# FarrOutLab/GWInferno

Hardware: AMD Instinct MI355X
Metric: log-likelihood evals/sec (value + gradient + diagnostic sites, host theta -> host results) (higher is better)
Workload: dtype f64; 1 GPU; C2: PL+Peak m1 x PL q x PL z, 69 ev x 5000 PE x 50k inj; n_events=69, n_pe=5000, n_inj=50000, n_theta=6, parallelism=single GPU

## Files before the change

### gwinferno_amd/csrc/gwi_device.h

```cpp
#pragma once
#ifndef __HIPCC_RTC__
#include <hip/hip_runtime.h>
#endif

#include "gwi_engine.h"

namespace gwi {

constexpr int kBlock = 256;
constexpr int kWaves = kBlock / 64;
constexpr int kMaxDerived = 7;
constexpr int kRecHeader = 3;

struct TermD {
  int kind, n_basis;
  int th0, th1, th2, th3;
  int flags, th4;
  double p0, p1, p2;
  double p3;
};
static_assert(sizeof(TermD) == 64, "twelve of these sit in the 4 KiB kernel-argument block");

struct NormD {
  int n_pts, expo_theta, n_basis, coef_off, flags, pad;
// ... 897 lines not shown
  }
  __device__ static void init(Acc& a) {
#pragma unroll
    for (int j = 0; j < 5; ++j) a.g[j] = 0;
  }
  __device__ static void rescale(Acc& a, double sc) {
#pragma unroll
    for (int j = 0; j < 5; ++j) a.g[j] *= sc;
  }
  static constexpr int kNumAcc = 5;
  __device__ static void collect(const TermD& t, const Acc& a, double* vals, int* th) {
#pragma unroll
    for (int j = 0; j < 5; ++j) vals[j] = a.g[j];
    th[0] = t.th0;
    th[1] = t.th1;
    th[2] = t.th2;
    th[3] = t.th3;
    th[4] = t.th4;
  }
};

template <>
struct Absorbs<GWI_TERM_PLPEAK> {
  static constexpr bool value = true;
};
template <>
struct Absorbs<GWI_TERM_PLPEAK_SMOOTH> {
  static constexpr bool value = true;
};

template <>
struct Term<GWI_TERM_POWERLAW_BOUNDS> {
  static constexpr bool kSpline = false;
  struct In {
    double x0, x1;
  };
  __device__ static void load(const double* const* tc, SIdx idx, In& in) {
    in.x0 = gload(tc[0], idx);
    in.x1 = gload(tc[1], idx);
  }
  struct State {
    double lx;
  };
  struct Acc {
    double g0;
  };
  __device__ static double eval(const TermD& t, const double*, const Ctx& c, const In& in, State& s, double& lin) {
    s.lx = in.x0;
    if ((in.x1 < c.theta[t.th1]) || (in.x1 > c.theta[t.th2])) {
      lin = 0.0;
      s.lx = 0.0;
    }
    return c.theta[t.th0] * s.lx;
  }
  __device__ static void accumulate(const TermD&, const Ctx&, double w, const State& s, Acc& a) { a.g0 += w * s.lx; }
  GWI_ACC1(g0)
  static constexpr int kNumAcc = 1;
  __device__ static void collect(const TermD& t, const Acc& a, double* vals, int* th) {
    vals[0] = a.g0;
    th[0] = t.th0;
  }
};

template <>
struct Term<GWI_TERM_EXP_SPLINE_LERP> {
  static constexpr bool kSpline = true;
  struct In {
    double x0;
  };
  __device__ static void load(const double* const* tc, SIdx idx, In& in) { in.x0 = gload(tc[0], idx); }
  struct State {
    double t0, t1, f;
    int k0, k1;
  };
  struct Acc {};
  __device__ static double node(const TermD& t, const Ctx& c, double sx, double wt, int& k, double& tt, double& lin) {
    spline_locate_x(sx, t, k, tt);
    double v = spline_value(c, t.th0 + k, tt);
    if (!((sx >= t.p0) && (sx <= t.p1))) {
      k = -1;
      v = 0.0;
      if (!(t.flags & GWI_SPLINE_OUTSIDE_ZERO_EXPONENT) && wt != 0.0) lin = 0.0;
    }
    if (wt == 0.0) k = -1;
    return v;
  }
  __device__ static double eval(const TermD& t, const double*, const Ctx& c, const In& in, State& s, double& lin) {
    const NormD& nd = c.a->norms[t.th1];
    const double u = in.x0;
    int j = (int)u;
    j = max(0, min(j, nd.n_pts - 2));
    const double f = u - (double)j;
    const double s0 = gload(nd.us, j), s1 = gload(nd.us, j + 1);
    const double l0 = node(t, c, s0, 1.0 - f, s.k0, s.t0, lin);
    const double l1 = node(t, c, s1, f, s.k1, s.t1, lin);
    s.f = f;
    return fma(f, l1 - l0, l0);
  }
  __device__ static void accumulate(const TermD& t, const Ctx& c, double w, const State& s, Acc&) {
    if (w != 0.0) {
      if (s.k0 >= 0) spline_scatter(c, t.th0 + s.k0, cubic_taps_weighted(s.t0, make_weight(w * (1.0 - s.f))));
      if (s.k1 >= 0) spline_scatter(c, t.th0 + s.k1, cubic_taps_weighted(s.t1, make_weight(w * s.f)));
    }
  }
  __device__ static void init(Acc&) {}
  __device__ static void rescale(Acc&, double) {}
  static constexpr int kNumAcc = 0;
  __device__ static void collect(const TermD&, const Acc&, double*, int*) {}
};

template <int U, bool TAKEN, int... Ks>
struct ChainImpl;
template <int U, bool TAKEN>
struct ChainImpl<U, TAKEN> {
  static constexpr bool kGeneric = false;
  static constexpr bool kSpline = false;
  static constexpr bool kAbsorb = false;
  static constexpr int kNumAcc = 0;
  __device__ void init() {}
  __device__ void load(int, int, int, const Ctx&, SIdx) {}
  __device__ void advance() {}
  __device__ double eval(int, int, const Ctx&, double&) { return 0.0; }
  __device__ double finish(int, int, const Ctx&, double, double, int) { return 0.0; }
  __device__ void accumulate(int, int, const Ctx&, double, double) {}
  __device__ void rescale(double) {}
  __device__ void collect(int, const Ctx&, double*, int*) {}
};
template <int U, bool TAKEN, int K, int... Rest>
struct ChainImpl<U, TAKEN, K, Rest...> {
  static constexpr bool kDefer = !TAKEN && Absorbs<K>::value;
  using RestT = ChainImpl<U, TAKEN || kDefer, Rest...>;
  static constexpr bool kGeneric = false;
  static constexpr bool kSpline = Term<K>::kSpline || RestT::kSpline;
  static constexpr bool kAbsorb = kDefer || RestT::kAbsorb;
  static constexpr int kNumAcc = Term<K>::kNumAcc + RestT::kNumAcc;
  typename Term<K>::In in[2][U];
  typename Term<K>::State st[U];
  typename Term<K>::Acc acc;
  RestT rest;
  __device__ void init() {
    Term<K>::init(acc);
    rest.init();
  }
  __device__ void load(int buf, int u, int ti, const Ctx& c, SIdx idx) {
    Term<K>::load(c.tcols[ti], idx, in[buf][u]);
    rest.load(buf, u, ti + 1, c, idx);
  }
  __device__ void advance() {
#pragma unroll
    for (int u = 0; u < U; ++u) in[0][u] = in[1][u];
    rest.advance();
  }
  __device__ double eval(int u, int ti, const Ctx& c, double& lin) {
    if constexpr (kDefer) {
      return rest.eval(u, ti + 1, c, lin);
    } else {
      const double l = Term<K>::eval(c.a->terms[ti], c.derived[ti], c, in[0][u], st[u], lin);
      return l + rest.eval(u, ti + 1, c, lin);
    }
  }
  __device__ double finish(int u, int ti, const Ctx& c, double L, double E, int nshift) {
    if constexpr (kDefer)
      return Term<K>::finish(c.a->terms[ti], c.derived[ti], c, in[0][u], st[u], L, E, nshift);
    else
      return rest.finish(u, ti + 1, c, L, E, nshift);
  }
  __device__ void accumulate(int u, int ti, const Ctx& c, double w, double wfac) {
    if constexpr (kDefer)
      Term<K>::accumulate_weighted(wfac, st[u], acc);
    else
      Term<K>::accumulate(c.a->terms[ti], c, w, st[u], acc);
    rest.accumulate(u, ti + 1, c, w, wfac);
  }
  __device__ void rescale(double sc) {
    Term<K>::rescale(acc, sc);
    rest.rescale(sc);
  }
  __device__ void collect(int ti, const Ctx& c, double* vals, int* th) {
    Term<K>::collect(c.a->terms[ti], acc, vals, th);
    rest.collect(ti + 1, c, vals + Term<K>::kNumAcc, th + Term<K>::kNumAcc);
  }
};

constexpr int kGenericChain = 0;
#define GWI_FOR_EACH_KIND(X)                                                                                             \
  X(GWI_TERM_POWERLAW) X(GWI_TERM_PLPEAK) X(GWI_TERM_POWERLAW_RATIO) X(GWI_TERM_BETA) X(GWI_TERM_TILT_MIXTURE)           \
  X(GWI_TERM_POWERLAW_REDSHIFT) X(GWI_TERM_EXP_SPLINE) X(GWI_TERM_TRUNCNORM) X(GWI_TERM_LINEAR_SPLINE) X(GWI_TERM_TILT_JOINT) \
  X(GWI_TERM_SMOOTH) X(GWI_TERM_PLPEAK_SMOOTH) X(GWI_TERM_POWERLAW_BOUNDS) X(GWI_TERM_EXP_SPLINE_LERP) X(GWI_TERM_EXP_SPLINE_F32)        \
  X(GWI_TERM_LINEAR_SPLINE_F32)
template <int K>
__device__ __forceinline__ double generic_value(const TermD& t, const double* d, const Ctx& c, const double* const* tc, SIdx idx, double& lin) {
  typename Term<K>::In in;
  typename Term<K>::State st;
  Term<K>::load(tc, idx, in);
  return Term<K>::eval(t, d, c, in, st, lin);
}
template <int K>
__device__ __forceinline__ void generic_gradient(const TermD& t, const double* d, const Ctx& c, const double* const* tc, SIdx idx, double w) {
  typename Term<K>::In in;
  typename Term<K>::State st;
  typename Term<K>::Acc acc;
  Term<K>::load(tc, idx, in);
  double lin = 1.0;
  Term<K>::eval(t, d, c, in, st, lin);
  Term<K>::init(acc);
  Term<K>::accumulate(t, c, w, st, acc);
  constexpr int kN = Term<K>::kNumAcc;
  if constexpr (kN > 0) {
    double vals[kN];
    int th[kN];
    Term<K>::collect(t, acc, vals, th);
#pragma unroll
    for (int j = 0; j < kN; ++j)
      if (vals[j] != 0.0) unsafeAtomicAdd(c.gacc + (th[j] << c.rep_shift), vals[j]);
  }
}
template <int U>
struct ChainImpl<U, false, kGenericChain> {
  static constexpr bool kGeneric = true;
  static constexpr bool kSpline = true;
  static constexpr bool kAbsorb = false;
  static constexpr int kNumAcc = 0;
  SIdx idx[2][U];
  __device__ void init() {}
  __device__ void load(int buf, int u, int, const Ctx&, SIdx i) { idx[buf][u] = i; }
  __device__ void advance() {
#pragma unroll
    for (int u = 0; u < U; ++u) idx[0][u] = idx[1][u];
  }
  __device__ double eval(int u, int, const Ctx& c, double& lin) {
    double l = 0.0;
    for (int t = 0; t < c.a->n_terms; ++t) {
      const TermD& td = c.a->terms[t];
      switch (td.kind) {
#define GWI_X(K) \
  case K: l += generic_value<K>(td, c.derived[t], c, c.tcols[t], idx[0][u], lin); break;
        GWI_FOR_EACH_KIND(GWI_X)
#undef GWI_X
        default: lin = 0.0;
      }
    }
    return l;
  }
  __device__ double finish(int, int, const Ctx&, double, double, int) { return 0.0; }
  __device__ void accumulate(int u, int, const Ctx& c, double w, double) {
    if (w == 0.0) return;
    c.wt = make_weight(w);
    for (int t = 0; t < c.a->n_terms; ++t) {
      const TermD& td = c.a->terms[t];
      switch (td.kind) {
#define GWI_X(K) \
  case K: generic_gradient<K>(td, c.derived[t], c, c.tcols[t], idx[0][u], w); break;
        GWI_FOR_EACH_KIND(GWI_X)
#undef GWI_X
        default: break;
      }
    }
  }
  __device__ void rescale(double) {}
  __device__ void collect(int, const Ctx&, double*, int*) {}
};

template <int U, int... Ks>
using Chain = ChainImpl<U, false, Ks...>;


__device__ __forceinline__ void store_sys(double* p, double v) { __hip_atomic_store(p, v, __ATOMIC_RELAXED, __HIP_MEMORY_SCOPE_SYSTEM); }
__device__ __forceinline__ void publish_stamp(double* slot, unsigned long long seq, int tid) {
  asm volatile("s_waitcnt vmcnt(0)" ::: "memory");
  __syncthreads();
  if (tid == 0) __hip_atomic_store(reinterpret_cast<unsigned long long*>(slot), seq, __ATOMIC_RELAXED, __HIP_MEMORY_SCOPE_SYSTEM);
}
__device__ __forceinline__ double lane_bcast(double v, int src) {
  const int lo = __builtin_amdgcn_readlane(__double2loint(v), src);
  const int hi = __builtin_amdgcn_readlane(__double2hiint(v), src);
  return __hiloint2double(hi, lo);
}

__device__ __forceinline__ double load_fresh(const double* p) { return __hip_atomic_load(p, __ATOMIC_RELAXED, __HIP_MEMORY_SCOPE_SYSTEM); }
__device__ __forceinline__ void combine_group(const TailArgs& a, const int e, const int kb, const int tid) {
  const int lane = tid & 63;
  const bool is_inj = e >= a.n_ev;
  int n_tiles;
  long long first;
  if (is_inj) {
    const int j = e - a.n_ev;
    const int t0 = j * a.tiles_per_inj_group;
    n_tiles = a.n_inj_tiles - t0 < a.tiles_per_inj_group ? a.n_inj_tiles - t0 : a.tiles_per_inj_group;
    first = (long long)a.n_ev * a.tiles_per_event + t0;
  } else {
    n_tiles = a.tiles_per_event;
    first = (long long)e * a.tiles_per_event;
  }
  const int n_groups = a.n_ev + a.n_inj_groups;
  const double* rec = a.partials + ((long long)kb * a.n_scan_blocks + first) * a.rec_stride;
  double* const ev_out = a.ev_out + (long long)kb * a.n_ev * 4;
  double* const ev_grad = a.ev_grad + (long long)kb * a.n_ev * a.n_theta;
  double* const inj_out = a.inj_out + (long long)kb * a.n_inj_groups * 4;
  double* const inj_grad = a.inj_grad + (long long)kb * a.n_inj_groups * a.n_theta;
  double* const ev_host = a.ev_host + (long long)kb * 3 * a.n_ev;
  const int row_doubles = 8 * a.row_lines;
  double* const host_rows = a.host_rows ? a.host_rows + (long long)kb * n_groups * row_doubles : nullptr;
  __shared__ double s_row[4 + GWI_MAX_THETA];

  const bool has = lane < n_tiles;
  const double* mine = rec + (long long)(has ? lane : 0) * a.rec_stride;
  const double m_t = has ? load_fresh(mine) : GWI_NEG_INF;
  const double r1 = has ? load_fresh(mine + 1) : 0.0, r2 = has ? load_fresh(mine + 2) : 0.0;
  constexpr int kEarly = 16;
  double early[kEarly];
  const bool early_on = tid < a.n_theta;
  {
    const double* col0 = rec + kRecHeader + (early_on ? tid : 0);
#pragma unroll
    for (int t = 0; t < kEarly; ++t) early[t] = (early_on && t < n_tiles) ? load_fresh(col0 + (long long)t * a.rec_stride) : 0.0;
  }
  const double M = wave_max(m_t);
  const double f = (m_t == GWI_NEG_INF) ? 0.0 : exp(m_t - M);
  const double S1 = wave_sum(f * r1);
  const double inv_s1 = S1 > 0.0 ? 1.0 / S1 : 0.0;
  for (int p = tid; p < a.n_theta; p += a.combine_threads) {
    double acc = 0.0;
    const double* col = rec + kRecHeader + p;
    int t = 0;
    if (p == tid) {
#pragma unroll
      for (; t < kEarly; ++t)
        if (t < n_tiles) acc += lane_bcast(f, t) * early[t];
      t = n_tiles < kEarly ? n_tiles : kEarly;
    }
#pragma unroll 4
    for (; t < n_tiles; ++t) acc += lane_bcast(f, t) * load_fresh(col + (long long)t * a.rec_stride);
    if (host_rows)
      s_row[3 + p] = is_inj ? acc : acc * inv_s1;
    else if (is_inj)
      inj_grad[(long long)(e - a.n_ev) * a.n_theta + p] = acc;
    else
      ev_grad[(long long)e * a.n_theta + p] = acc * inv_s1;
  }
  if (tid < 64) {
    const double S2 = wave_sum(f * f * r2);
    if (lane == 0 && host_rows) {
      if (is_inj) {
        s_row[0] = M;
        s_row[1] = S1;
        s_row[2] = S2;
      } else {
        const double log_s1 = log(S1);
        const double log_neff = 2.0 * log_s1 - log(S2);
        s_row[0] = log_s1 + M;
        s_row[1] = log_neff;
        s_row[2] = 1.0 / exp(log_neff) - 1.0 / a.n_pe;
      }
    } else if (lane == 0) {
      if (is_inj) {
        double* o = inj_out + (long long)(e - a.n_ev) * 4;
        o[0] = M;
        o[1] = S1;
        o[2] = S2;
      } else {
        const double log_s1 = log(S1);
        const double log_neff = 2.0 * log_s1 - log(S2);
        const double var = 1.0 / exp(log_neff) - 1.0 / a.n_pe;
        double* o = ev_out + (long long)e * 4;
        o[0] = log_s1 + M;
        o[1] = log_neff;
        o[2] = var;
        o[3] = S1;
        if (a.publish_events) {
          store_sys(ev_host + e, log_s1 + M);
          store_sys(ev_host + a.n_ev + e, log_neff);
          store_sys(ev_host + 2 * a.n_ev + e, var);
        }
      }
    }
  }
  if (host_rows) {
    __syncthreads();
    unsigned long long* o = reinterpret_cast<unsigned long long*>(host_rows + (long long)e * row_doubles);
    const unsigned long long seq = __hip_atomic_load(a.seq_ptr, __ATOMIC_RELAXED, __HIP_MEMORY_SCOPE_SYSTEM);
    const int n_vals = 3 + a.n_theta;
    for (int slot = tid; slot < row_doubles; slot += a.combine_threads) {
      const int line = slot >> 3, j = slot & 7, i = line * 7 + j;
      const unsigned long long bits = j == 7 ? seq : (i < n_vals ? (unsigned long long)__double_as_longlong(s_row[i]) : 0ull);
      __hip_atomic_store(o + slot, bits, __ATOMIC_RELAXED, __HIP_MEMORY_SCOPE_SYSTEM);
    }
  }
}

__device__ __forceinline__ int pow2_at_least(int v) {
  int p = 1;
  while (p < v) p <<= 1;
  return p;
}

template <int THREADS>
__device__ __forceinline__ void final_reduce(const TailArgs& a, const int kb, const int g, const int tid, double* s_tile ) {
  const int lane = tid & 63, wave = tid >> 6;
  const int G = a.final_groups;
  const int e_lo = (int)((long long)g * a.n_ev / G), e_hi = (int)((long long)(g + 1) * a.n_ev / G);
  const int j_lo = (int)((long long)g * a.n_inj_groups / G), j_hi = (int)((long long)(g + 1) * a.n_inj_groups / G);
  const int n_ig = j_hi - j_lo;
  double* r = a.record + ((long long)kb * G + g) * a.record_len;
  const double* const ev_out = a.ev_out + (long long)kb * a.n_ev * 4;
  const double* const ev_grad = a.ev_grad + (long long)kb * a.n_ev * a.n_theta;
  const double* const inj_out = a.inj_out + ((long long)kb * a.n_inj_groups + j_lo) * 4;
  const double* const inj_grad = a.inj_grad + ((long long)kb * a.n_inj_groups + j_lo) * a.n_theta;
  const int off_norm = 8, off_gpe = off_norm + a.n_norms, off_ginj = off_gpe + a.n_theta;

  const int vp = pow2_at_least(a.n_theta < 8 ? 8 : a.n_theta);
  const int rows = THREADS / vp;
  const int row = tid / vp, col = tid - row * vp;
  double acc = 0.0;
  if (col < a.n_theta) {
    for (int e0 = e_lo + row; e0 < e_hi; e0 += 16 * rows) {
      double v[16];
#pragma unroll
      for (int q = 0; q < 16; ++q) {
        const int e = e0 + q * rows;
        v[q] = e < e_hi ? ev_grad[(long long)e * a.n_theta + col] : 0.0;
      }
#pragma unroll
      for (int q = 0; q < 16; ++q) acc += v[q];
    }
  }
  s_tile[tid] = acc;

  if (wave == 0) {
    double sum = 0.0, var = 0.0, mn = GWI_POS_INF;
    for (int e0 = e_lo + lane; e0 < e_hi; e0 += 4 * 64) {
      double o0[4], o1[4], o2[4];
#pragma unroll
      for (int q = 0; q < 4; ++q) {
        const int e = e0 + 64 * q;
        const double* o = ev_out + (long long)(e < e_hi ? e : e_lo) * 4;
        o0[q] = o[0];
        o1[q] = o[1];
        o2[q] = o[2];
      }
#pragma unroll
      for (int q = 0; q < 4; ++q) {
        if (e0 + 64 * q >= e_hi) continue;
        sum += o0[q];
        var += o2[q];
        double le = o1[q];
        if (le != le) le = 0.0;
        le = fmin(fmax(le, -1.7976931348623157e308), 1.7976931348623157e308);
        mn = fmin(mn, le);
      }
    }
    sum = wave_sum(sum);
    var = wave_sum(var);
    mn = -wave_max(-mn);
    if (lane == 0) {
      store_sys(r + 1, sum);
      store_sys(r + 2, var);
      store_sys(r + 3, mn);
      store_sys(r + 7, (*a.redo_ptr == *a.seq_ptr) ? -(double)(e_hi - e_lo + 1) : (double)(e_hi - e_lo));
    }
  }
  const bool hasg = lane < n_ig;
  const double m_j = hasg ? inj_out[lane * 4] : GWI_NEG_INF;
  const double s1_j = hasg ? inj_out[lane * 4 + 1] : 0.0, s2_j = hasg ? inj_out[lane * 4 + 2] : 0.0;
  constexpr int kEarly = 32;
  double early[kEarly];
  const bool early_on = tid < a.n_theta;
#pragma unroll
  for (int j = 0; j < kEarly; ++j) early[j] = (early_on && j < n_ig) ? inj_grad[(long long)j * a.n_theta + tid] : 0.0;
  const double Minj = wave_max(m_j);
  const double fj = (m_j == GWI_NEG_INF) ? 0.0 : exp(m_j - Minj);
  if (wave == 1) {
    const double S1 = wave_sum(fj * s1_j);
    const double S2 = wave_sum(fj * fj * s2_j);
    if (lane == 0) {
      store_sys(r + 4, Minj);
      store_sys(r + 5, S1);
      store_sys(r + 6, S2);
    }
  }
  for (int p = tid; p < a.n_theta; p += THREADS) {
    double gsum = 0.0;
    int j = 0;
    if (p == tid) {
#pragma unroll
      for (; j < kEarly; ++j)
        if (j < n_ig) gsum += lane_bcast(fj, j) * early[j];
      j = n_ig < kEarly ? n_ig : kEarly;
    }
    for (; j < n_ig; j += 8) {
      double v[8];
#pragma unroll
      for (int q = 0; q < 8; ++q) v[q] = (j + q < n_ig) ? inj_grad[(long long)(j + q) * a.n_theta + p] : 0.0;
#pragma unroll
      for (int q = 0; q < 8; ++q)
        if (j + q < n_ig) gsum += lane_bcast(fj, j + q) * v[q];
    }
    store_sys(r + off_ginj + p, gsum);
  }
  __syncthreads();
  if (row == 0 && col < a.n_theta) {
    double gsum = 0.0;
    for (int q = 0; q < rows; ++q) gsum += s_tile[q * vp + col];
    store_sys(r + off_gpe + col, gsum);
  }
  publish_stamp(r, *a.seq_ptr, tid);
}

__device__ __forceinline__ void norm_block(const NormD* norms, const double* theta_src, int n_theta, int j, double* out_slot, unsigned long long* stamp_slot,
                                           unsigned long long seq, double* s_theta, double* s_part ) {
  const int tid = threadIdx.x;
  for (int p = tid; p < n_theta; p += kBlock) s_theta[p] = theta_src[p];
  __syncthreads();
  const NormD nd = norms[j];
  double acc = 0.0;
  const double expo = nd.expo_theta >= 0 ? s_theta[nd.expo_theta] + nd.expo_add : 0.0;
  const double inv_dx = nd.n_basis > 0 ? (double)(nd.n_basis - 3) / (nd.hi - nd.lo) : 0.0;
  for (int g = tid; g < nd.n_pts; g += kBlock) {
    const double tw = nd.tw[g];
    double e = nd.lb ? nd.lb[g] : 0.0;
    if (nd.expo_theta >= 0) e += expo * nd.l1[g];
    if (nd.n_basis > 0) {
      const double x = nd.us[g];
      int k;
      double tt;
      spline_locate(x, nd.lo, inv_dx, nd.n_basis, k, tt);
      const Taps b = cubic_taps(tt);
      const double* cf = s_theta + nd.coef_off + k;
      double v = cf[0] * b.b0 + cf[1] * b.b1 + cf[2] * b.b2 + cf[3] * b.b3;
      if ((nd.flags & (GWI_SPLINE_OUTSIDE_ZERO_EXPONENT | GWI_NORM_LINEAR_SPLINE)) && !((x >= nd.lo) && (x <= nd.hi))) v = 0.0;
      if (nd.flags & GWI_NORM_LINEAR_SPLINE) {
        acc += tw * v;
        continue;
      }
      e += v;
    }
    if (tw != 0.0) acc += tw * fast_exp(e);
  }
  acc = wave_sum(acc);
  if ((tid & 63) == 0) s_part[tid >> 6] = acc;
  __syncthreads();
  if (tid == 0) store_sys(out_slot, (s_part[0] + s_part[1]) + (s_part[2] + s_part[3]));
  asm volatile("s_waitcnt vmcnt(0)" ::: "memory");
  __syncthreads();
  if (tid == 0) __hip_atomic_store(stamp_slot, seq, __ATOMIC_RELAXED, __HIP_MEMORY_SCOPE_SYSTEM);
}

constexpr int kHeadCols = 5;
struct ScanHead {
  const double* col[kHeadCols];
  unsigned geom;
  unsigned chunks;
  unsigned n_pe, n_inj;
};
static_assert(sizeof(ScanHead) == 56, "fourteen dwords: what the command processor preloads next to the kernel-argument pointer");
constexpr unsigned kGeomEventBits = 20, kGeomTilesBits = 7;
__host__ __device__ inline bool chunk_packs(long long c) { return c > 0 && (c < 32768 || (c % 256 == 0 && c / 256 < 32768)); }
__host__ __device__ inline unsigned pack_chunk(long long c) { return c < 32768 ? (unsigned)c : (0x8000u | (unsigned)(c / 256)); }
__host__ __device__ inline int unpack_chunk(unsigned v) { return (v & 0x8000u) ? (int)((v & 0x7fffu) * 256u) : (int)v; }
__host__ __device__ inline long long inj_offset(long long n_ev, long long n_pe) { return (n_ev * n_pe + 31) / 32 * 32; }

template <int SLOT, int T, int... Ks>
struct ColFill;
template <int SLOT, int T>
struct ColFill<SLOT, T> {
  __device__ static void run(const double* (*)[2], const double* const*, const KArgs&) {}
};
template <int SLOT, int T, int K, int... Rest>
struct ColFill<SLOT, T, K, Rest...> {
  static constexpr int kCols = (int)(sizeof(typename Term<K>::In) / sizeof(double));
  __device__ __forceinline__ static void run(const double* (*lc)[2], const double* const* head, const KArgs& a) {
#pragma unroll
    for (int k = 0; k < 2; ++k) lc[T][k] = k < kCols ? (SLOT + k < kHeadCols ? head[SLOT + k < kHeadCols ? SLOT + k : 0] : a.pe_tcols[T][k]) : nullptr;
    ColFill<SLOT + kCols, T + 1, Rest...>::run(lc, head, a);
  }
};

template <int N_TERMS, bool BATCHED>
struct KernargWarm {
  static constexpr int kRanges = 4;
  static constexpr size_t lo(int r) {
    return r == 0 ? offsetof(KArgs, pe_tcols) : r == 1 ? offsetof(KArgs, kappa_pe) : r == 2 ? offsetof(KArgs, norm_seq) : offsetof(KArgs, theta);
  }
  static constexpr size_t hi(int r) {
    return r == 0   ? offsetof(KArgs, pe_tcols) + 16 * N_TERMS
           : r == 1 ? offsetof(KArgs, terms) + sizeof(TermD) * N_TERMS
           : r == 2 ? offsetof(KArgs, derived) + sizeof(double) * kMaxDerived * N_TERMS
                    : offsetof(KArgs, theta) + 128;
  }
  static constexpr int count() {
    int n = 0;
    for (int r = 0; r < kRanges; ++r)
      for (size_t o = lo(r) & ~(size_t)63; o < hi(r); o += 64) ++n;
    return n;
  }
  static constexpr size_t offset(int k) {
    int n = 0;
    for (int r = 0; r < kRanges; ++r)
      for (size_t o = lo(r) & ~(size_t)63; o < hi(r); o += 64) {
        if (n == k) return o;
        ++n;
      }
    return 0;
  }
  static constexpr int kN = BATCHED ? 0 : count();
  int t[kN > 0 ? kN : 1];
  __device__ __forceinline__ void issue() {
    const char __attribute__((address_space(4)))* w = (const char __attribute__((address_space(4)))*)__builtin_amdgcn_kernarg_segment_ptr() + sizeof(ScanHead);
#pragma unroll
    for (int k = 0; k < kN; ++k) asm volatile("s_load_dword %0, %1, 0x0" : "=&s"(t[k]) : "s"(w + offset(k)));
  }
  __device__ __forceinline__ void settle() {
    if (kN > 0) asm volatile("s_waitcnt lgkmcnt(0)" ::: "memory");
#pragma unroll
    for (int k = 0; k < kN; ++k) asm volatile("" ::"s"(t[k]));
  }
};

struct TileGeom {
  int n_norms, tiles, n_ev, chunk_pe, chunk_inj;
  long long n_pe, n_inj;
  __device__ __forceinline__ static TileGeom decode(unsigned h_geom, unsigned h_chunks, unsigned hu_n_pe, unsigned hu_n_inj) {
    TileGeom g;
    g.n_norms = (int)(h_geom >> (kGeomEventBits + kGeomTilesBits)), g.tiles = (int)((h_geom >> kGeomEventBits) & ((1u << kGeomTilesBits) - 1u));
    g.n_ev = (int)(h_geom & ((1u << kGeomEventBits) - 1u));
    g.chunk_pe = unpack_chunk(h_chunks & 0xffffu), g.chunk_inj = unpack_chunk(h_chunks >> 16);
    g.n_pe = hu_n_pe, g.n_inj = hu_n_inj;
    return g;
  }
};

__device__ __forceinline__ void stamp_sequence(unsigned long long seq, unsigned long long* seq_dev) { *seq_dev = seq; }

__device__ __forceinline__ int binades_of(double mm) { return (int)__builtin_rint(fmin(fmax(mm, -7.0e5), 7.0e5) * kLog2e); }

__device__ __forceinline__ bool positive_finite(double s) { return s > 0.0 && s < GWI_POS_INF; }

constexpr int kRegularRepShift = 4;

#ifndef GWI_SCAN_WAVES_PER_EU
#define GWI_SCAN_WAVES_PER_EU 1
#endif
template <bool WRITE_LOGW, bool BATCH, bool SAFE, int U, int... Ks>
__global__ __launch_bounds__(kBlock, GWI_SCAN_WAVES_PER_EU) void scan_kernel(const double* hc0, const double* hc1, const double* hc2, const double* hc3, const double* hc4, const unsigned h_geom,
                                                                             const unsigned h_chunks, const unsigned hu_n_pe, const unsigned hu_n_inj, const KArgs a) {
  using ChainT = Chain<U, Ks...>;
  constexpr int kU = U;
  constexpr bool kShared = ChainT::kSpline && !WRITE_LOGW;
  extern __shared__ double s_gacc[];
  __shared__ double s_theta[GWI_MAX_THETA];
  __shared__ double s_out[GWI_MAX_THETA];
  constexpr int kNVals = 2 + ChainT::kNumAcc;
  constexpr int kSumGroups = (kNVals + 7) / 8;
  __shared__ double s_part[kWaves][kSumGroups * 8];
  __shared__ double s_wrec[kWaves][4];
  const int tid = threadIdx.x, lane = tid & 63, wave = tid >> 6;
#ifdef GWI_STAMPS
  unsigned long long stamp_v[8] = {0, 0, 0, 0, 0, 0, 0, 0};
#define GWI_STAMP(k)                                                                                   \
  do {                                                                                                 \
    stamp_v[k] = __builtin_amdgcn_s_memrealtime();                                                     \
    if ((k) == 4 && lane == 0) {                                                                       \
      unsigned long long* stamp_row_ = a.stamps + ((long long)blockIdx.x * kWaves + wave) * 8;         \
      for (int q_ = 0; q_ < 8; ++q_) stamp_row_[q_] = stamp_v[q_];                                     \
    }                                                                                                  \
  } while (0)
#else
#define GWI_STAMP(k) \
  do {               \
  } while (0)
#endif
  GWI_STAMP(0);
#ifdef GWI_STAMPS
  {
    unsigned hw_id, xcc_id;
    asm volatile("s_getreg_b32 %0, hwreg(HW_REG_HW_ID)" : "=s"(hw_id));
    asm volatile("s_getreg_b32 %0, hwreg(HW_REG_XCC_ID)" : "=s"(xcc_id));
    stamp_v[5] = ((unsigned long long)xcc_id << 32) | hw_id;
  }
#endif
  const TileGeom geom = TileGeom::decode(h_geom, h_chunks, hu_n_pe, hu_n_inj);
  const int kb = (BATCH || SAFE) ? (int)blockIdx.y : 0;
  const int n_norm_blocks = WRITE_LOGW ? 0 : geom.n_norms;
  if ((int)blockIdx.x < n_norm_blocks) {
    const bool batch_n = BATCH || (SAFE && a.tblocks != nullptr);
    const int j = blockIdx.x;
    if (blockIdx.x == 0 && kb == 0 && tid == 0) stamp_sequence(a.norm_seq, a.seq_dev);
    norm_block(a.norms, batch_n ? a.tblocks[kb].theta : a.theta, a.n_theta, j, a.norm_out_host + kb * geom.n_norms + j, a.norm_stamps_host + kb * geom.n_norms + j, a.norm_seq, s_theta, &s_wrec[0][0]);
    return;
// ... 569 lines not shown
```

Before: 64880 evals/s.

## Assign host-row value runs per wave to replace block barrier with wave barrier

In the combine path that writes host rows, each wave now computes exactly the theta gradient values that fall into its own 9-line run of the host row. That wave then writes those lines itself, so the block-wide __syncthreads becomes a wavefront fence plus wave barrier. The sequence-number load is hoisted to the start of the kernel so its latency overlaps the record loads. The S2/header computation is split so wave 0 writes the header before the gradient loop. With n_theta=6 every value sits in wave 0's run, so the gain is mostly the removed block barrier and the earlier seq load. The risk is a subtle ordering bug if any value were produced by a different wave than the one writing it.

```diff
diff --git a/gwinferno_amd/csrc/gwi_device.h b/gwinferno_amd/csrc/gwi_device.h
--- a/gwinferno_amd/csrc/gwi_device.h
+++ b/gwinferno_amd/csrc/gwi_device.h
@@ -1223,16 +1223,22 @@
   const int row_doubles = 8 * a.row_lines;
   double* const host_rows = a.host_rows ? a.host_rows + (long long)kb * n_groups * row_doubles : nullptr;
   __shared__ double s_row[4 + GWI_MAX_THETA];
+  unsigned long long seq = 0;
+  if (host_rows) seq = __hip_atomic_load(a.seq_ptr, __ATOMIC_RELAXED, __HIP_MEMORY_SCOPE_SYSTEM);
 
   const bool has = lane < n_tiles;
   const double* mine = rec + (long long)(has ? lane : 0) * a.rec_stride;
   const double m_t = has ? load_fresh(mine) : GWI_NEG_INF;
   const double r1 = has ? load_fresh(mine + 1) : 0.0, r2 = has ? load_fresh(mine + 2) : 0.0;
+  constexpr int kRunLines = 9, kRunVals = 7 * kRunLines;
+  const int wave = tid >> 6, n_waves = a.combine_threads >> 6;
+  const int p0 = !host_rows ? tid : (lane < kRunVals ? kRunVals * wave + lane - 3 : a.n_theta);
+  const int p_step = host_rows ? kRunVals * n_waves : a.combine_threads;
   constexpr int kEarly = 16;
   double early[kEarly];
-  const bool early_on = tid < a.n_theta;
+  const bool early_on = p0 >= 0 && p0 < a.n_theta;
   {
-    const double* col0 = rec + kRecHeader + (early_on ? tid : 0);
+    const double* col0 = rec + kRecHeader + (early_on ? p0 : 0);
 #pragma unroll
     for (int t = 0; t < kEarly; ++t) early[t] = (early_on && t < n_tiles) ? load_fresh(col0 + (long long)t * a.rec_stride) : 0.0;
   }
@@ -1240,28 +1246,9 @@
   const double f = (m_t == GWI_NEG_INF) ? 0.0 : exp(m_t - M);
   const double S1 = wave_sum(f * r1);
   const double inv_s1 = S1 > 0.0 ? 1.0 / S1 : 0.0;
-  for (int p = tid; p < a.n_theta; p += a.combine_threads) {
-    double acc = 0.0;
-    const double* col = rec + kRecHeader + p;
-    int t = 0;
-    if (p == tid) {
-#pragma unroll
-      for (; t < kEarly; ++t)
-        if (t < n_tiles) acc += lane_bcast(f, t) * early[t];
-      t = n_tiles < kEarly ? n_tiles : kEarly;
-    }
-#pragma unroll 4
-    for (; t < n_tiles; ++t) acc += lane_bcast(f, t) * load_fresh(col + (long long)t * a.rec_stride);
-    if (host_rows)
-      s_row[3 + p] = is_inj ? acc : acc * inv_s1;
-    else if (is_inj)
-      inj_grad[(long long)(e - a.n_ev) * a.n_theta + p] = acc;
-    else
-      ev_grad[(long long)e * a.n_theta + p] = acc * inv_s1;
-  }
-  if (tid < 64) {
+  if (tid < 64 && host_rows) {
     const double S2 = wave_sum(f * f * r2);
-    if (lane == 0 && host_rows) {
+    if (lane == 0) {
       if (is_inj) {
         s_row[0] = M;
         s_row[1] = S1;
@@ -1273,7 +1260,31 @@
         s_row[1] = log_neff;
         s_row[2] = 1.0 / exp(log_neff) - 1.0 / a.n_pe;
       }
-    } else if (lane == 0) {
+    }
+  }
+  for (int p = p0; p < a.n_theta; p += p_step) {
+    if (p < 0) continue;
+    double acc = 0.0;
+    const double* col = rec + kRecHeader + p;
+    int t = 0;
+    if (p == p0) {
+#pragma unroll
+      for (; t < kEarly; ++t)
+        if (t < n_tiles) acc += lane_bcast(f, t) * early[t];
+      t = n_tiles < kEarly ? n_tiles : kEarly;
+    }
+#pragma unroll 4
+    for (; t < n_tiles; ++t) acc += lane_bcast(f, t) * load_fresh(col + (long long)t * a.rec_stride);
+    if (host_rows)
+      s_row[3 + p] = is_inj ? acc : acc * inv_s1;
+    else if (is_inj)
+      inj_grad[(long long)(e - a.n_ev) * a.n_theta + p] = acc;
+    else
+      ev_grad[(long long)e * a.n_theta + p] = acc * inv_s1;
+  }
+  if (tid < 64 && !host_rows) {
+    const double S2 = wave_sum(f * f * r2);
+    if (lane == 0) {
       if (is_inj) {
         double* o = inj_out + (long long)(e - a.n_ev) * 4;
         o[0] = M;
@@ -1297,14 +1308,19 @@
     }
   }
   if (host_rows) {
-    __syncthreads();
+    __builtin_amdgcn_fence(__ATOMIC_RELEASE, "wavefront");
+    __builtin_amdgcn_wave_barrier();
     unsigned long long* o = reinterpret_cast<unsigned long long*>(host_rows + (long long)e * row_doubles);
-    const unsigned long long seq = __hip_atomic_load(a.seq_ptr, __ATOMIC_RELAXED, __HIP_MEMORY_SCOPE_SYSTEM);
     const int n_vals = 3 + a.n_theta;
-    for (int slot = tid; slot < row_doubles; slot += a.combine_threads) {
-      const int line = slot >> 3, j = slot & 7, i = line * 7 + j;
-      const unsigned long long bits = j == 7 ? seq : (i < n_vals ? (unsigned long long)__double_as_longlong(s_row[i]) : 0ull);
-      __hip_atomic_store(o + slot, bits, __ATOMIC_RELAXED, __HIP_MEMORY_SCOPE_SYSTEM);
+    for (int run = wave; run * kRunLines < a.row_lines; run += n_waves) {
+#pragma unroll
+      for (int s = lane; s < 8 * kRunLines; s += 64) {
+        const int slot = 8 * kRunLines * run + s;
+        if (slot >= row_doubles) break;
+        const int line = slot >> 3, j = slot & 7, i = line * 7 + j;
+        const unsigned long long bits = j == 7 ? seq : (i < n_vals ? (unsigned long long)__double_as_longlong(s_row[i]) : 0ull);
+        __hip_atomic_store(o + slot, bits, __ATOMIC_RELAXED, __HIP_MEMORY_SCOPE_SYSTEM);
+      }
     }
   }
 }
```

After: 63790 evals/s. -1.7%, worse.
